# verificatum/verificatum-vmn

Hardware: AMD Instinct MI355X
Metric: modexps/sec (batched variable-base modPow, 2048-bit ModPGroup, full-length exponents) (higher is better)
Workload: dtype u32 limbs (28-bit radix), u64 accumulate

## Files before the change

__graft_entry__.py:

```python
from __future__ import annotations

import importlib.util
import os
import subprocess
import sys

ROOT = os.path.dirname(os.path.abspath(__file__))
PKG_DIR = os.path.join(ROOT, "verificatum-vmn_amd")
CSRC = os.path.join(PKG_DIR, "csrc")
LIB = os.path.join(PKG_DIR, "libvmnhip.so")
PROOFS_LIB = os.path.join(PKG_DIR, "libvmnproofs.so")


def load_package():
    name = "verificatum_vmn_amd"
    if name in sys.modules:
        return sys.modules[name]
    spec = importlib.util.spec_from_file_location(name, os.path.join(PKG_DIR, "__init__.py"),
                                                  submodule_search_locations=[PKG_DIR])
    mod = importlib.util.module_from_spec(spec)
    sys.modules[name] = mod
    spec.loader.exec_module(mod)
    return mod


def _newer(target: str, sources) -> bool:
    if not os.path.exists(target):
        return False
    t = os.path.getmtime(target)
    return all(os.path.getmtime(s) <= t for s in sources)


def build() -> None:
    hipcc = os.environ.get("HIPCC", "/opt/rocm/bin/hipcc")
    gspec = importlib.util.spec_from_file_location("gen_mont_asm", os.path.join(ROOT, "tools", "gen_mont_asm.py"))
    gmod = importlib.util.module_from_spec(gspec)
    gspec.loader.exec_module(gmod)
    gen = gmod.render([10, 14, 19, 37, 74], [110], [148, 76, 112], [80, 296], [592])
    inc = os.path.join(CSRC, "gen", "mont_rows.inc")
    inc29 = os.path.join(CSRC, "gen", "mont29_rows.inc")
    for path, text in ((inc, gen), (inc29, gmod.render29([71]))):
        if not os.path.exists(path) or open(path).read() != text:
            with open(path, "w") as f:
                f.write(text)
    units = ("vmnhip.hip", "inst_small.hip", "inst_2048.hip", "inst_2048_short.hip", "inst_2048_wide.hip", "inst_3072.hip", "inst_4096.hip", "inst_8192.hip",
             "inst_16384.hip", "inst_p224.hip", "inst_p256.hip", "inst_p384.hip", "inst_p521.hip",
             "inst_g9.hip", "inst_g10.hip", "inst_g13.hip", "inst_g15.hip", "inst_g21.hip")
    sources = [os.path.join(CSRC, f) for f in units + ("modp_kernels.h", "modp_shared_exp.h", "modp_instances.h", "ec_instances.h", "light_kernels.h", "ec_kernels.h", "mont28.h", "hostbig.h", "expprod_schedule.h", "ec_shared_schedule.h", "hexlines_layout.h", "jsonlines_layout.h", "decimal_kernels.h",
                                                       "vmnhip_internal.h", "sha256.h", "sha512.h", "hostnum64.h", "hosttrace.h")]
    sources += [inc, inc29, os.path.join(ROOT, "include", "vmnhip.h")]
    if not _newer(LIB, sources):
        objdir = os.path.join(CSRC, "build")
        os.makedirs(objdir, exist_ok=True)
        procs = []
        for u in units:
            obj = os.path.join(objdir, u.replace(".hip", ".o"))
            cmd = [hipcc, "-std=c++20", "-O3", "--offload-arch=gfx950", "-fPIC", "-c", os.path.join(CSRC, u), "-o", obj]
            procs.append((cmd, obj, subprocess.Popen(cmd)))
        objs = []
        for cmd, obj, pr in procs:
            if pr.wait() != 0:
                for _, _, other in procs:
                    if other.poll() is None:
                        other.kill()
                raise subprocess.CalledProcessError(pr.returncode, cmd)
            objs.append(obj)
        subprocess.run([hipcc, "--offload-arch=gfx950", "-shared", "-o", LIB] + objs, check=True)
    psrc = [os.path.join(CSRC, "vmnproofs.cpp"), os.path.join(CSRC, "hostnum64.h"), os.path.join(CSRC, "hostcurve.h"), os.path.join(CSRC, "hosttrace.h"),
            os.path.join(ROOT, "include", "vmnproofs.h"),
            os.path.join(ROOT, "include", "vmnhip.h"), LIB]
    if not _newer(PROOFS_LIB, psrc):
        subprocess.run(["g++", "-std=c++17", "-O2", "-Wall", "-pthread", "-fPIC", "-shared", os.path.join(CSRC, "vmnproofs.cpp"), "-o", PROOFS_LIB,
                        "-L" + PKG_DIR, "-lvmnhip", "-Wl,-rpath,$ORIGIN"], check=True)
    orc_dir = os.path.join(ROOT, "oracle")
    if not _newer(os.path.join(orc_dir, "libvmnoracle.so"), [os.path.join(orc_dir, "vmn_oracle.c")]):
        subprocess.run(["make", "-B", "-C", orc_dir, "libvmnoracle.so"], check=True,
                       stdout=subprocess.PIPE, stderr=subprocess.STDOUT)
    load_package()


def smoke() -> None:
    if ROOT not in sys.path:
        sys.path.insert(0, ROOT)
    vmn = load_package()
    from oracle import pyref
    from oracle.cbind import Oracle

    p, q, g = pyref.modp_group(2048)
    n = 512
    xs = [pow(1 + v % (p - 1), 2, p) for v in pyref.stream_ints(b"smoke/x", n, p)]
    es = pyref.stream_ints(b"smoke/e", n, q)
    ctx = vmn.Context(0)
    grp = vmn.ModPGroup(ctx, p, q, g)
    X = grp.toElementArray(xs)
    E = grp.ringArray(es)
    got = X.exp(E).toInts()
    orc = Oracle(p, q)
    want = orc.exp_array(xs, es)
    assert got == want, "smoke: HIP modpow differs from the GMP oracle"
    got_fixed = grp.exp(g, E).toInts()
    assert got_fixed == orc.exp_fixed(g, es), "smoke: HIP fixed-base exp differs from the GMP oracle"
# ... 40 lines not shown
```

verificatum-vmn_amd/csrc/modp_instances.h:

```cpp
#pragma once
#include "modp_kernels.h"
#include "modp_shared_exp.h"

#define VMN_MODP_INSTANCES(KW, S_, NW_, LPE_)                                                                                          \
    KW __global__ void vmn::k_import_be<vmn::Cfg<S_, LPE_>, NW_>(vmn::u32*, const uint8_t*, size_t, size_t, int, size_t, const vmn::u32*, \
                                                                 vmn::u32, const vmn::u32*, vmn::u32*);                                   \
    KW __global__ void vmn::k_export_be<vmn::Cfg<S_, LPE_>, NW_>(uint8_t*, size_t, size_t, int, const vmn::u32*, size_t, const vmn::u32*, \
                                                                 vmn::u32);                                                               \
    KW __global__ void vmn::k_to_words<vmn::Cfg<S_, LPE_>, NW_>(vmn::u32*, const vmn::u32*, size_t, const vmn::u32*, vmn::u32);           \
    KW __global__ void vmn::k_mul<vmn::Cfg<S_, LPE_>>(vmn::u32*, const vmn::u32*, const vmn::u32*, size_t, size_t, const vmn::u32*,      \
                                                      vmn::u32);                                                                         \
    KW __global__ void vmn::k_modpow<vmn::Cfg<S_, LPE_>>(vmn::u32*, const vmn::u32*, const vmn::u32*, int, size_t, int, int, size_t,     \
                                                         const vmn::u32*, vmn::u32, const vmn::u32*, vmn::u32*);                         \
    KW __global__ void vmn::k_modpow_phased<vmn::Cfg<S_, LPE_>>(vmn::u32*, const vmn::u32*, const vmn::u32*, int, size_t, int, int,      \
                                                                size_t, const vmn::u32*, vmn::u32, const vmn::u32*, vmn::u32*, int,      \
                                                                vmn::u32*, vmn::u32*);                                                   \
    KW __global__ void vmn::k_modpow2<vmn::Cfg<S_, LPE_>>(vmn::u32*, const vmn::u32*, const vmn::u32*, int, size_t, int, const vmn::u32*,  \
                                                          const vmn::u32*, int, size_t, int, int, size_t, const vmn::u32*, vmn::u32,      \
                                                          const vmn::u32*, vmn::u32*);                                                  \
    KW __global__ void vmn::k_modpow2_phased<vmn::Cfg<S_, LPE_>>(vmn::u32*, const vmn::u32*, const vmn::u32*, int, size_t, int,          \
                                                                 const vmn::u32*, const vmn::u32*, int, size_t, int, int, size_t,        \
                                                                 const vmn::u32*, vmn::u32, const vmn::u32*, vmn::u32*, int, vmn::u32*,  \
                                                                 vmn::u32*);                                                            \
    KW __global__ void vmn::k_modpow_shared<vmn::Cfg<S_, LPE_>>(vmn::u32*, const vmn::u32*, const vmn::SlideStep*, int, int, size_t,      \
                                                                const vmn::u32*, vmn::u32, vmn::u32*);                                  \
    KW __global__ void vmn::k_modpow_shared_phased<vmn::Cfg<S_, LPE_>>(vmn::u32*, const vmn::u32*, const vmn::SlideStep*, int, int,      \
                                                                       size_t, const vmn::u32*, vmn::u32, vmn::u32*, int, vmn::u32*,     \
                                                                       vmn::u32*);                                                      \
    KW __global__ void vmn::k_modpow_shared_multi<vmn::Cfg<S_, LPE_>>(vmn::SharedArrays, vmn::u32, vmn::u32, const vmn::SlideStep*, int,  \
                                                                      int, size_t, const vmn::u32*, vmn::u32, vmn::u32*);              \
    KW __global__ void vmn::k_modpow_shared_multi_phased<vmn::Cfg<S_, LPE_>>(vmn::SharedArrays, vmn::u32, vmn::u32,                     \
                                                                             const vmn::SlideStep*, int, int, size_t, const vmn::u32*,  \
                                                                             vmn::u32, vmn::u32*, int, vmn::u32*, vmn::u32*);           \
    KW __global__ void vmn::k_modpow_shared_each<vmn::Cfg<S_, LPE_>>(vmn::EachArrays, vmn::u32, vmn::u32, const vmn::SlideStep*, int,     \
                                                                     size_t, const vmn::u32*, vmn::u32, vmn::u32*);                    \
    KW __global__ void vmn::k_modpow_shared_each_phased<vmn::Cfg<S_, LPE_>>(vmn::EachArrays, vmn::u32, vmn::u32, const vmn::SlideStep*,  \
                                                                            int, size_t, const vmn::u32*, vmn::u32, vmn::u32*, int,    \
                                                                            vmn::u32*, vmn::u32*);                                     \
    KW __global__ void vmn::k_modpow_expprod<vmn::Cfg<S_, LPE_>>(vmn::ExpProdArrays, vmn::u32, vmn::u32, const vmn::SlideStep*, vmn::u32,    \
                                                                 const vmn::u32*, vmn::u32, vmn::u32*);                                \
    KW __global__ void vmn::k_modpow_jobs<vmn::Cfg<S_, LPE_>>(vmn::ModpowJob, vmn::ModpowJob, unsigned, int, const vmn::u32*, vmn::u32,    \
                                                              const vmn::u32*, vmn::u32*);                                             \
    KW __global__ void vmn::k_reduce_strided<vmn::Cfg<S_, LPE_>, true>(vmn::u32*, const vmn::u32*, size_t, size_t, size_t,               \
                                                                       const vmn::u32*, vmn::u32);                                       \
    KW __global__ void vmn::k_reduce_strided<vmn::Cfg<S_, LPE_>, false>(vmn::u32*, const vmn::u32*, size_t, size_t, size_t,              \
                                                                        const vmn::u32*, vmn::u32);                                      \
    KW __global__ void vmn::k_ring_elementwise<vmn::Cfg<S_, LPE_>>(vmn::u32*, const vmn::u32*, const vmn::u32*, const vmn::u32*, int,    \
                                                                   size_t, const vmn::u32*, vmn::u32);                                   \
    KW __global__ void vmn::k_scan_totals<vmn::Cfg<S_, LPE_>, true>(vmn::u32*, const vmn::u32*, const vmn::u32*, size_t, size_t, size_t, \
                                                                    int, const vmn::u32*, vmn::u32, const vmn::u32*);                    \
    KW __global__ void vmn::k_scan_totals<vmn::Cfg<S_, LPE_>, false>(vmn::u32*, const vmn::u32*, const vmn::u32*, size_t, size_t, size_t, \
                                                                     int, const vmn::u32*, vmn::u32, const vmn::u32*);                   \
    KW __global__ void vmn::k_scan_apply<vmn::Cfg<S_, LPE_>>(vmn::u32*, const vmn::u32*, const vmn::u32*, const vmn::u32*, size_t,       \
                                                             size_t, size_t, int, const vmn::u32*, vmn::u32, const vmn::u32*);           \
    KW __global__ void vmn::k_fixed_level<vmn::Cfg<S_, LPE_>>(vmn::u32*, int, int, int, const vmn::u32*, vmn::u32);                      \
    KW __global__ void vmn::k_fixed_exp<vmn::Cfg<S_, LPE_>>(vmn::u32*, const vmn::u32*, int, int, const vmn::u32*, int, size_t, int,     \
                                                            const vmn::u32*, vmn::u32);                                                  \
    KW __global__ void vmn::k_bucket_level<vmn::Cfg<S_, LPE_>, true>(vmn::u32*, size_t, vmn::LevelInputs, unsigned, const vmn::u32*,     \
                                                                     const vmn::u32*, const vmn::u32*, const vmn::u32*, size_t, size_t, \
                                                                     vmn::u32, const vmn::u32*, vmn::u32);                               \
    KW __global__ void vmn::k_bucket_level<vmn::Cfg<S_, LPE_>, false>(vmn::u32*, size_t, vmn::LevelInputs, unsigned, const vmn::u32*,    \
                                                                      const vmn::u32*, const vmn::u32*, const vmn::u32*, size_t, size_t, \
                                                                      vmn::u32, const vmn::u32*, vmn::u32);

#define VMN_MEMBER_INSTANCE_ONE_LANE(KW, S_, LPE_) \
    KW __global__ void vmn::k_jacobi_member<vmn::Cfg<S_, LPE_>>(const vmn::u32*, size_t, const vmn::u32*, vmn::u32*);
#define VMN_MEMBER_INSTANCE_LANES(KW, S_, LPE_) \
    KW __global__ void vmn::k_jacobi_member_lanes<vmn::Cfg<S_, LPE_>>(const vmn::u32*, size_t, const vmn::u32*, vmn::u32*);

#define VMN_UNIT_SMALL(KW)                                                                                             \
    VMN_MODP_INSTANCES(KW, 10, 8, 1) VMN_MODP_INSTANCES(KW, 14, 12, 1) VMN_MODP_INSTANCES(KW, 19, 16, 1)                 \
    VMN_MODP_INSTANCES(KW, 37, 32, 1) VMN_MEMBER_INSTANCE_ONE_LANE(KW, 10, 1) VMN_MEMBER_INSTANCE_ONE_LANE(KW, 14, 1)     \
    VMN_MEMBER_INSTANCE_ONE_LANE(KW, 19, 1) VMN_MEMBER_INSTANCE_ONE_LANE(KW, 37, 1)
#define VMN_UNIT_2048(KW) VMN_MODP_INSTANCES(KW, 74, 64, 1) VMN_MEMBER_INSTANCE_ONE_LANE(KW, 74, 1)
#define VMN_UNIT_2048_SHORT(KW)                                                                                        \
    KW __global__ void vmn::k_modpow<vmn::Cfg<74, 1>, true>(vmn::u32*, const vmn::u32*, const vmn::u32*, int, size_t, int, int, size_t, \
                                                            const vmn::u32*, vmn::u32, const vmn::u32*, vmn::u32*);                     \
    KW __global__ void vmn::k_modpow_phased<vmn::Cfg<74, 1>, true>(vmn::u32*, const vmn::u32*, const vmn::u32*, int, size_t, int, int,  \
                                                                   size_t, const vmn::u32*, vmn::u32, const vmn::u32*, vmn::u32*, int,  \
                                                                   vmn::u32*, vmn::u32*);
#define VMN_UNIT_2048_WIDE(KW)                                                                                         \
    VMN_MODP_INSTANCES(KW, 76, 64, 4) VMN_MODP_INSTANCES(KW, 80, 64, 8)                                                \
    KW __global__ void vmn::k_modpow_jobs_mixed<vmn::Cfg<80, 8>, vmn::Cfg<76, 4>>(vmn::ModpowJob, vmn::ModpowJob, unsigned, int,       \
                                                                                 const vmn::u32*, vmn::u32, const vmn::u32*, vmn::u32*);
#define VMN_UNIT_3072(KW) VMN_MODP_INSTANCES(KW, 110, 96, 2) VMN_MODP_INSTANCES(KW, 112, 96, 4) VMN_MEMBER_INSTANCE_LANES(KW, 110, 2)
#define VMN_UNIT_4096(KW) VMN_MODP_INSTANCES(KW, 148, 128, 4) VMN_MEMBER_INSTANCE_LANES(KW, 148, 4)
#define VMN_UNIT_8192(KW) VMN_MODP_INSTANCES(KW, 296, 256, 8) VMN_MEMBER_INSTANCE_LANES(KW, 296, 8)
#define VMN_UNIT_16384(KW) VMN_MODP_INSTANCES(KW, 592, 512, 16) VMN_MEMBER_INSTANCE_LANES(KW, 592, 16)
```

verificatum-vmn_amd/csrc/vmnhip.hip:

```cpp
#include <stdarg.h>

#include <algorithm>
#include <future>
#include <memory>
#include <system_error>
#include <utility>

#include "ec_kernels.h"
#include "modp_kernels.h"
#include "modp_instances.h"
#include "ec_instances.h"
#include "light_kernels.h"
#include "decimal_kernels.h"
#include "vmnhip_internal.h"
#include "sha256.h"
#include "sha512.h"
#include "hostnum64.h"
#include "ec_shared_schedule.h"
#include "expprod_schedule.h"
#include "hexlines_layout.h"

VMN_UNIT_SMALL(extern template)
VMN_UNIT_2048(extern template)
VMN_UNIT_2048_SHORT(extern template)
VMN_UNIT_2048_WIDE(extern template)
VMN_UNIT_3072(extern template)
VMN_UNIT_4096(extern template)
VMN_UNIT_8192(extern template)
VMN_UNIT_16384(extern template)
VMN_UNIT_P224(extern template)
VMN_UNIT_P256(extern template)
VMN_UNIT_P384(extern template)
VMN_UNIT_P521(extern template)
VMN_UNIT_G9(extern template)
VMN_UNIT_G10(extern template)
VMN_UNIT_G13(extern template)
VMN_UNIT_G15(extern template)
VMN_UNIT_G21(extern template)

using namespace vmn;
using vmn::hostbig::Big;

static thread_local char g_err[512] = "";
void vmn::set_error(const char* fmt, ...) {
    va_list ap;
    va_start(ap, fmt);
    vsnprintf(g_err, sizeof(g_err), fmt, ap);
    va_end(ap);
}
extern "C" const char* vmn_last_error(void) { return g_err; }
static thread_local vmn_ctx* tl_helper_of = nullptr;
vmn_ctx* vmn::lane_of(vmn_ctx* c) { return (c && tl_helper_of == c && c->helper) ? c->helper : c; }
extern "C" void vmn_report_error(const char* message) { vmn::set_error("%s", message ? message : ""); }
extern "C" const char* vmn_version(void) { return "vmnhip 0.1 (gfx950, radix-2^28 lazy-carry Montgomery)"; }

#define ARG_CHECK(cond, msg)             \
    do {                                 \
        if (!(cond)) {                   \
// ... 26 lines not shown
static int with_curve(const vmn_modulus& m, F&& f) {
#define X(S_, NW_, K_) \
    if (m.ec->S == S_ && m.ec->kind == K_) return f(CurveCfg<S_, NW_, K_>{});
    VMN_FOR_CURVES(X)
#undef X
    return VMN_ERR_ARG;
}

static bool size_for_bits(int nbits, int* S, int* NW, int* LPE) {
    const int sizes[][4] = {{256, 10, 8, 1}, {384, 14, 12, 1}, {512, 19, 16, 1}, {1024, 37, 32, 1}, {2048, 74, 64, 1},
                            {3072, 110, 96, 2}, {4096, 148, 128, 4}, {8192, 296, 256, 8}, {16384, 592, 512, 16}};
    for (auto& s : sizes) {
        if (nbits <= s[0]) {
            *S = s[1];
            *NW = s[2];
            *LPE = s[3];
            return true;
        }
    }
    return false;
}

static size_t default_wide_max() {
    static const size_t v = [] {
        const char* env = getenv("VMN_WIDE_MAX");
        return env ? (size_t)strtoull(env, nullptr, 10) : (size_t)40960;
    }();
    return v;
}
static size_t default_wide8_max() {
    static const size_t v = [] {
        const char* env = getenv("VMN_WIDE8_MAX");
        return env ? (size_t)strtoull(env, nullptr, 10) : (size_t)6144;
    }();
    return v;
}
static size_t fixed_split_fill() {
    const char* env = getenv("VMN_FIXED_SPLIT_FILL");
    return env ? (size_t)strtoull(env, nullptr, 10) : (size_t)786432;
}
static const vmn_modulus& geom(const vmn_ctx* ctx, const vmn_modulus& m, size_t items, bool always = false) {
    const vmn_ctx* root = ctx->parent ? ctx->parent : ctx;
    if (m.wide8 && root->wide8_max != 0 && (items <= root->wide8_max || (always && items <= root->wide_max))) return *m.wide8;
    if (!m.wide || root->wide_max == 0) return m;
    return (always || items <= root->wide_max) ? *m.wide : m;
}
template <class F>
static int with_geom(const vmn_ctx* ctx, const vmn_modulus& m0, size_t items, F&& f, bool always = false) {
    const vmn_modulus& m = geom(ctx, m0, items, always);
    return with_cfg(m, [&](auto c, auto w) { return f(c, w, m); });
}
static size_t lds_bytes(const vmn_modulus& m) { return (size_t)m.S * (BLOCK / m.LPE) * sizeof(u32); }
static int blocks_per_cu(const vmn_modulus&) { return 2; }

template <typename... KArgs, typename... Args>
static int launch_timed(vmn_ctx* ctx, const char* family, void (*kernel)(KArgs...), unsigned grid, size_t lds, Args... args) {
    TimingRec rec;
    if (ctx->timing) {
        rec.family = family;
        rec.mads = ctx->next_mads;
        rec.canon = ctx->next_canon;
        VMN_HIP(hipEventCreate(&rec.start));
        VMN_HIP(hipEventCreate(&rec.stop));
        VMN_HIP(hipEventRecord(rec.start, ctx->stream));
    }
    ctx->next_mads = ctx->next_canon = 0;
    hipLaunchKernelGGL(kernel, dim3(grid), dim3(BLOCK), lds, ctx->stream, static_cast<KArgs>(args)...);
    VMN_HIP(hipGetLastError());
    if (ctx->timing) {
        VMN_HIP(hipEventRecord(rec.stop, ctx->stream));
        ctx->recs.push_back(rec);
    }
    return VMN_OK;
}
template <typename... KArgs, typename... Args>
static int launch(vmn_ctx* ctx, const char* family, void (*kernel)(KArgs...), unsigned grid, size_t lds, Args... args) {
    const void* kp = reinterpret_cast<const void*>(kernel);
    if (!ctx->lds_attr_set.count(kp)) {
        VMN_HIP(hipFuncSetAttribute(kp, hipFuncAttributeMaxDynamicSharedMemorySize, (int)lds));
        ctx->lds_attr_set.insert(kp);
    }
    return launch_timed(ctx, family, kernel, grid, lds, args...);
}

static void note_work(vmn_ctx* ctx, const vmn_modulus& m, double products, double squarings = 0, double canon_products = -1) {
    if (!ctx->timing) return;
    const double S = m.ec ? (double)m.ec->S : (double)m.S;
    const double Rw = m.ec ? S : (double)m.rows;
    const double s32 = (double)((m.nbits + 31) / 32);
    ctx->next_canon = (canon_products >= 0 ? canon_products : products) * (2 * s32 * s32 + s32) +
                      squarings * (m.ec ? 2 * s32 * s32 + s32 : s32 * (s32 + 1) / 2 + s32 * s32 + s32);
    if (m.ec) {
        const bool known = m.ec->kind == EC_NIST;
        const double nz = known && m.ec->S == 10 ? 7 : known && m.ec->S == 15 ? 12 : S;
        ctx->next_mads = (products + squarings) * (S * S + S * nz);
        return;
    }
    const double sq = Rw * S + Rw * (S + SQR_BLK * m.LPE) / 2;
    ctx->next_mads = products * 2 * Rw * S + squarings * sq;
}
static const double EC_ADD = 15.4, EC_MADD = 10.6, EC_DBL = 6.9, EC_NORM = 7.0, EC_INV = 380;
static const double EC_MADD_RUN = 9.7;

static unsigned light_grid(vmn_ctx* ctx, size_t work_items) {
    size_t blocks = (work_items + BLOCK - 1) / BLOCK;
    size_t cap = (size_t)ctx->num_cus * 8;
// ... 1338 lines not shown
    int phases = 1;
    DevTmp tab, sync_words;
    PhasePlan(vmn_ctx* ctx, const vmn_modulus& m, size_t n, size_t arrays = 1)
        : max_blocks((unsigned)(ctx->num_cus * blocks_per_cu(m))), epb((size_t)(BLOCK / m.LPE)), ntiles(arrays * ((n + epb - 1) / epb)),
          tab(ctx), sync_words(ctx) {
        if (const char* mb = getenv("VMN_MODPOW_MAX_BLOCKS")) {
            const int v = atoi(mb);
            if (v >= 1) max_blocks = std::min<unsigned>(max_blocks, (unsigned)v);
        }
        grid = (unsigned)std::min<size_t>(ntiles, max_blocks);
    }
    size_t slot_tables_bytes(const vmn_modulus& m, size_t rows) const { return (size_t)grid * epb * rows * elem_words(m) * sizeof(uint32_t); }
    int split(vmn_ctx* ctx, const vmn_modulus& m, int cuttable_steps, size_t rows) {
        static const int phases_env = [] {
            const char* e = getenv("VMN_MODPOW_PHASES");
            return e && *e ? std::max(1, atoi(e)) : 16;
        }();
        if (ntiles <= (size_t)max_blocks || ntiles >= ((size_t)1 << 26)) return VMN_OK;
        const int want = std::min(phases_env, std::max(1, cuttable_steps));
        const size_t tab_bytes = ntiles * epb * rows * elem_words(m) * sizeof(uint32_t);
        if (want == 1 || tab_bytes > ((size_t)64 << 30) || tab.alloc(tab_bytes) != VMN_OK) return VMN_OK;
        VMN_TRY(sync_words.alloc((ntiles + 1) * sizeof(uint32_t)));
        VMN_TRY(dev_zero(ctx, sync_words.p, (ntiles + 1) * sizeof(uint32_t)));
        phases = want;
        return VMN_OK;
    }
    uint32_t* table() { return tab.as<uint32_t>(); }
    uint32_t* queue() { return sync_words.as<uint32_t>(); }
    uint32_t* done() { return queue() + 1; }
};

static int modpow_words(vmn_ctx* ctx, const vmn_modulus& m0, const uint32_t* x, const uint32_t* e_words, int ewords,
                        size_t estride, int ebits, size_t n, uint32_t* out) {
    if (n == 0) return VMN_OK;
    if (ebits < 1) ebits = 1;
    if (m0.ec) {
        const vmn_modulus& m = m0;
        int wb = std::min(pick_window(ebits), 5);
        unsigned grid = std::min<unsigned>(grid_for(n), (unsigned)(ctx->num_cus * 2));
        size_t tab_bytes = (size_t)grid * BLOCK * ((size_t)1 << wb) * elem_words(m) * sizeof(uint32_t);
        VMN_TRY(ensure_scratch(ctx, tab_bytes));
        note_work(ctx, m, (double)n * (EC_DBL * ebits + EC_ADD * ((ebits + wb - 1) / wb + (1 << wb))));
        return with_curve(m, [&]<class E>(E) {
            return launch_light(ctx, "modpow", k_ec_mulvar<E::S, E::KIND>, grid, out, x, e_words, ewords, estride, ebits, wb, n, ecdev(m.ec),
                                reinterpret_cast<uint32_t*>(ctx->scratch));
        });
    }
    int wbits = pick_window(ebits);
    const vmn_modulus& m = geom(ctx, m0, n);
    const int nwin = (ebits + wbits - 1) / wbits;
    PhasePlan pl(ctx, m, n);
    VMN_TRY(ensure_scratch(ctx, pl.slot_tables_bytes(m, (size_t)1 << wbits)));
    note_work(ctx, m, (double)n * (nwin - 1 + (1 << wbits) - 2), (double)n * (nwin - 1) * wbits);
    const bool pow29 = m.S == 74 && m.LPE == 1;
    const char* short_env = getenv("VMN_POW29_SHORT");
    const bool pow29_short = pow29 && m.pow29_short && !(short_env && *short_env && atoi(short_env) == 0);
    if (pow29 && ctx->timing) {
        const double S9 = Cfg29::S, relief = 2 * (S9 - 2), red = S9 * (pow29_short ? S9 - 2 : S9);
        ctx->next_mads = (double)n * ((nwin - 1 + (1 << wbits) - 2 + 2) * (S9 * S9 + red + relief) +
                                      (double)(nwin - 1) * wbits * (red + S9 * (S9 + SQR_BLK) / 2 + relief));
    }
    VMN_TRY(pl.split(ctx, m, nwin - 1, (size_t)1 << wbits));
    static_assert(POW29<Cfg<74, 1>>, "modpow_words passes the 29-bit constants to the kernels of Cfg<74, 1>");
    const uint32_t* d_n = pow29 ? m.d_pow29 + (size_t)(pow29_short ? Cfg29::ROW_NS : Cfg29::ROW_N) * Cfg29::W : m.d_n;
    const uint32_t* d_one = pow29 ? m.d_pow29 + (size_t)Cfg29::ROW_ONE * Cfg29::W : m.d_one;
    const uint32_t n0inv = pow29 ? m.n0inv29 : m.n0inv;
    if (pow29_short) {
        using C = Cfg<74, 1>;
        if (pl.phases > 1)
            return launch(ctx, "modpow", k_modpow_phased<C, true>, pl.max_blocks, lds_bytes(m), out, x, e_words, ewords, estride, ebits,
                          wbits, n, d_n, n0inv, d_one, pl.table(), pl.phases, pl.queue(), pl.done());
        return launch(ctx, "modpow", k_modpow<C, true>, pl.grid, lds_bytes(m), out, x, e_words, ewords, estride, ebits, wbits, n, d_n,
                      n0inv, d_one, reinterpret_cast<uint32_t*>(ctx->scratch));
    }
    return with_cfg(m, [&]<class C, class W>(C, W) {
        if (pl.phases > 1)
            return launch(ctx, "modpow", k_modpow_phased<C>, pl.max_blocks, lds_bytes(m), out, x, e_words, ewords, estride, ebits, wbits, n,
                          d_n, n0inv, d_one, pl.table(), pl.phases, pl.queue(), pl.done());
        return launch(ctx, "modpow", k_modpow<C>, pl.grid, lds_bytes(m), out, x, e_words, ewords, estride, ebits, wbits, n, d_n, n0inv,
                      d_one, reinterpret_cast<uint32_t*>(ctx->scratch));
    });
}

static int sliding_window_bits(int ebits) {
    if (const char* env = getenv("VMN_SLIDING_WINDOW")) {
        int w = atoi(env);
        if (w >= 0 && w <= 8) return w;
    }
    int best = 2;
    long best_cost = 1L << 60;
    for (int w = 2; w <= 8; ++w) {
        long cost = (1L << (w - 1)) + ebits / (w + 1);
        if (cost < best_cost) {
            best_cost = cost;
            best = w;
        }
    }
    return best;
}
static void slide_schedule(const Big& e, int ebits, int w, std::vector<SlideStep>& steps, long& mults, long& squarings) {
    const size_t first = steps.size();
    int pending = 0;
    mults = squarings = 0;
    for (int i = ebits - 1; i >= 0;) {
        if (!hostbig::get_bit(e, i)) {
            ++pending;
            --i;
            continue;
        }
        int l = std::max(i - w + 1, 0);
        while (!hostbig::get_bit(e, l)) ++l;
        uint32_t val = 0;
        for (int b = i; b >= l; --b) val = (val << 1) | (uint32_t)hostbig::get_bit(e, b);
        steps.push_back(SlideStep{steps.size() == first ? 0 : pending + (i - l + 1), (int)((val - 1) / 2)});
        pending = 0;
        i = l - 1;
    }
    if (pending) steps.push_back(SlideStep{pending, -1});
// ... 2482 lines not shown
                                   (int)chain, ecdev(m.ec));
                return hipGetLastError() == hipSuccess ? VMN_OK : VMN_ERR_DEVICE;
            });
        }
        if (rc == VMN_OK)
            rc = launch_light(ctx, "fixed_table", k_fixed_seed, grid_for((size_t)nwin * (w + 1)), ft.d_tab,
                              (const uint32_t*)sq.as<uint32_t>(), w, nwin, (const uint32_t*)m.d_one, (int)Wd);
        for (int l = 1; l < w && rc == VMN_OK; ++l) {
            size_t lanes = (((size_t)1 << l) - 1) * nwin;
            rc = with_curve(m, [&]<class E>(E) {
                note_work(ctx, m, EC_ADD * (double)lanes);
                return launch_light(ctx, "fixed_table", k_ec_fixed_level<E::S, E::KIND>, grid_for(lanes), ft.d_tab, w, nwin, l, ecdev(m.ec));
            });
        }
        free_one(ctx, m, d_base);
        if (rc == VMN_OK) {
            DevTmp flat(ctx);
            const size_t entries = (size_t)nwin << w;
            rc = flat.alloc(entries * Wd * sizeof(uint32_t));
            const uint32_t* whole[1] = {ft.d_tab};
            if (rc == VMN_OK) rc = ec_normalize(ctx, m, whole, 1, entries, flat.as<uint32_t>());
            if (rc == VMN_OK && hipMemcpyAsync(ft.d_tab, flat.p, entries * Wd * sizeof(uint32_t), hipMemcpyDeviceToDevice, ctx->stream) != hipSuccess)
                rc = VMN_ERR_DEVICE;
        }
        if (rc != VMN_OK) {
            if (ft.d_tab) (void)hipFree(ft.d_tab);
            return rc;
        }
        ft.last_use = ++g->fixed_clock;
        ft.uses = carry_uses;
        ft.built_on = ctx->stream;
        if (hipEventCreateWithFlags(&ft.ready, hipEventDisableTiming) == hipSuccess) (void)hipEventRecord(ft.ready, ctx->stream);
        g->fixed_bytes += ft.bytes;
        auto ins = g->fixed.emplace(key, ft);
        *out = &ins.first->second;
        return VMN_OK;
    }
    VMN_TRACE("fixed_table:build");
    const size_t chain = (size_t)nwin * w;
    std::vector<uint8_t> own_chain;
    if (!chain_be || chain_be->size() != (chain + 1) * g->nbytes) {
        VMN_TRY(fixed_chain_host(g, base_be, chain, own_chain));
        chain_be = &own_chain;
    }
    const std::vector<uint8_t>& sq_be = *chain_be;
    DevTmp sq(ctx);
    VMN_TRY(sq.alloc((chain + 1) * Wd * sizeof(uint32_t)));
    int ok = 1;
    VMN_TRY(import_be(ctx, m, g->nbytes, sq_be.data(), chain + 1, sq.as<uint32_t>(), &ok));
    VMN_TRY(mul_arrays(ctx, m, sq.as<uint32_t>(), sq.as<uint32_t>() + chain * Wd, 0, chain, sq.as<uint32_t>()));
    vmn_group::FixedTable ft;
    ft.wbits = w;
    ft.nwin = nwin;
    ft.bytes = (size_t)nwin * ((size_t)1 << w) * Wd * sizeof(uint32_t);
    VMN_TRY(fixed_alloc(g, ft.bytes, &ft.d_tab));
    int rc = launch_light(ctx, "fixed_table", k_fixed_seed, grid_for((size_t)nwin * (w + 1)), ft.d_tab, (const uint32_t*)sq.as<uint32_t>(), w,
                          nwin, (const uint32_t*)m.d_one, (int)Wd);
    for (int l = 1; l < w && rc == VMN_OK; ++l) {
        size_t lanes = (((size_t)1 << l) - 1) * nwin;
        rc = with_geom(ctx, m, lanes, [&]<class C, class W>(C, W, const vmn_modulus& mg) {
            note_work(ctx, mg, (double)lanes);
            return launch(ctx, "fixed_table", k_fixed_level<C>, egrid(mg, lanes), lds_bytes(mg), ft.d_tab, w, nwin, l, mg.d_n, mg.n0inv);
        });
    }
    if (rc != VMN_OK) {
        (void)hipFree(ft.d_tab);
        return rc;
    }
    ft.last_use = ++g->fixed_clock;
    ft.uses = carry_uses;
    ft.built_on = ctx->stream;
    if (hipEventCreateWithFlags(&ft.ready, hipEventDisableTiming) == hipSuccess) (void)hipEventRecord(ft.ready, ctx->stream);
    g->fixed_bytes += ft.bytes;
    auto ins = g->fixed.emplace(key, ft);
    *out = &ins.first->second;
    return VMN_OK;
}

extern "C" int vmn_group_precompute_fixed(vmn_group* grp, const uint8_t* base_be, size_t n_hint, int uses_hint) {
    ARG_CHECK(grp && base_be && n_hint > 0, "bad argument");
    const int uses = uses_hint < 1 ? 1 : (uses_hint > 16 ? 16 : uses_hint);
    const int ebits = grp->Q.nbits;
    vmn_group::FixedTable* ft = nullptr;
    std::vector<uint8_t> chain;
    if (!grp->P.ec) {
        {
            VMN_ENTER(LANE(grp->ctx));
            std::lock_guard<std::recursive_mutex> tab_guard(grp->tab_mu);
            VMN_TRY(fixed_table(grp, base_be, ebits, n_hint, &ft, uses, true));
            if (ft) return VMN_OK;
        }
        const int w = fixed_window_for(grp, n_hint, ebits, uses);
        VMN_TRY(fixed_chain_host(grp, base_be, (size_t)((ebits + w - 1) / w) * w, chain));
    }
    VMN_ENTER(LANE(grp->ctx));
    std::lock_guard<std::recursive_mutex> tab_guard(grp->tab_mu);
    return fixed_table(grp, base_be, ebits, n_hint, &ft, uses, false, chain.empty() ? nullptr : &chain);
}

extern "C" int vmn_group_release_fixed(vmn_group* grp, const uint8_t* base_be) {
    ARG_CHECK(grp && base_be, "null argument");
    VMN_ENTER(LANE(grp->ctx));
    std::lock_guard<std::recursive_mutex> tab_guard(grp->tab_mu);
    std::string key(reinterpret_cast<const char*>(base_be), grp->P.ec ? 2 * grp->nbytes : grp->nbytes);
    auto it = grp->fixed.find(key);
    if (it != grp->fixed.end()) fixed_drop(grp, it);
    return VMN_OK;
}

extern "C" int vmn_group_exp_fixed(vmn_group* grp, const uint8_t* base_be, const vmn_rarray* e, vmn_garray** out) {
    ARG_CHECK(grp && base_be && e && out, "null argument");
    ARG_CHECK(e->grp == grp, "exponent array belongs to another group");
    vmn_ctx* ctx = LANE(grp->ctx);
    VMN_ENTER(ctx);
    const size_t n = e->n;
    vmn_garray* r = nullptr;
    VMN_TRY(new_garray(grp, n, &r));
    if (n == 0) {
        *out = r;
        return VMN_OK;
    }
    int ebits = grp->Q.nbits;
    vmn_group::FixedTable* ft = nullptr;
    DevTmp ew(ctx);
    std::lock_guard<std::recursive_mutex> tab_guard(grp->tab_mu);
    int rc = fixed_table(grp, base_be, ebits, n, &ft);
    if (rc == VMN_OK) rc = ew.alloc(n * (size_t)grp->Q.NW * sizeof(uint32_t));
    if (rc == VMN_OK) rc = to_words(ctx, grp->Q, e->d, n, ew.as<uint32_t>());
    if (rc == VMN_OK && grp->P.ec) {
        const vmn_modulus& m = grp->P;
        rc = with_curve(m, [&]<class E>(E) {
            note_work(ctx, m, EC_MADD_RUN * (double)n * (ft->nwin - 1), 0, EC_MADD * (double)n * (ft->nwin - 1));
            return launch_light(ctx, "fixed", k_ec_fixed_exp<E::S, E::KIND>, grid_for(n), r->d, (const uint32_t*)ft->d_tab, ft->wbits, ft->nwin,
                                (const uint32_t*)ew.as<uint32_t>(), grp->Q.NW, n, ecdev(m.ec));
        });
    } else if (rc == VMN_OK) {
        int parts = 1;
        const size_t fill = fixed_split_fill();
        while (parts < 16 && (size_t)(2 * parts) * n <= fill && ft->nwin / (2 * parts) >= 4) parts *= 2;
        const size_t items = n * (size_t)parts, Wd = elem_words(grp->P);
        const vmn_modulus& m = geom(ctx, grp->P, items);
        DevTmp pieces(ctx);
        if (parts > 1) rc = pieces.alloc(items * Wd * sizeof(uint32_t));
        uint32_t* dst = parts > 1 ? pieces.as<uint32_t>() : r->d;
        unsigned grid = egrid(m, items);
        if (rc == VMN_OK) {
            rc = with_cfg(m, [&]<class C, class W>(C, W) {
                note_work(ctx, m, (double)n * (ft->nwin - parts));
                return launch(ctx, "fixed", k_fixed_exp<C>, grid, lds_bytes(m), dst, (const uint32_t*)ft->d_tab, ft->wbits, ft->nwin,
                              (const uint32_t*)ew.as<uint32_t>(), grp->Q.NW, n, parts, m.d_n, m.n0inv);
            });
        }
        for (int half = parts / 2; half >= 1 && rc == VMN_OK; half /= 2) {
            uint32_t* lo = pieces.as<uint32_t>();
            rc = mul_arrays(ctx, grp->P, lo, lo + (size_t)half * n * Wd, Wd, (size_t)half * n, half == 1 ? r->d : lo);
        }
    }
    if (rc != VMN_OK) {
        vmn_garray_free(r);
        return rc;
    }
    *out = r;
    return VMN_OK;
}

static int ec_normalize(vmn_ctx* ctx, const vmn_modulus& m, const uint32_t* const* ins, size_t k, size_t n, uint32_t* out) {
    if (n == 0 || k == 0) return VMN_OK;
    const char* K_str = getenv("VMN_EC_NORMALISE_CHUNK");
    const size_t K_env = K_str && *K_str ? (size_t)std::max(2, atoi(K_str)) : (size_t)0;
    const size_t FWd = (size_t)stride_for_limbs(m.ec->S), Wd = (size_t)m.W, K = K_env ? K_env : 8, TOP = 2048;
    const size_t n1 = (n + K - 1) / K;
    std::vector<size_t> sizes{k * n, k * n1};
    while (sizes.back() > TOP) sizes.push_back((sizes.back() + K - 1) / K);
    const size_t L = sizes.size();
    size_t words = 0;
    std::vector<size_t> off_pref(L), off_val(L), off_inv(L);
    for (size_t l = 0; l < L; ++l) {
        off_pref[l] = words;
        words += (l + 1 < L ? sizes[l] : 0) * FWd;
        off_val[l] = words;
        words += (l > 0 ? sizes[l] : 0) * FWd;
        off_inv[l] = words;
        words += (l > 0 ? sizes[l] : 0) * FWd;
    }
    DevTmp buf(ctx);
    VMN_TRY(buf.alloc(words * sizeof(uint32_t)));
    uint32_t* B = buf.as<uint32_t>();
    double products = 7.0 * (double)(k * n) + EC_INV * (double)sizes[L - 1];
    for (size_t l = 1; l + 1 < L; ++l) products += 3.0 * (double)sizes[l];
    return with_curve(m, [&]<class E>(E) -> int {
        constexpr int S = E::S, KIND = E::KIND;
        note_work(ctx, m, products);
        const unsigned bpa = (unsigned)((n1 + BLOCK - 1) / BLOCK);
        for (size_t a0 = 0; a0 < k; a0 += LEVEL_ARRAYS) {
            const size_t ga = std::min<size_t>(LEVEL_ARRAYS, k - a0);
            LevelInputs li{};
            for (size_t a = 0; a < ga; ++a) li.p[a] = ins[a0 + a];
            VMN_TRY(launch_light(ctx, "normalize", k_finv_up<S, true, KIND>, (unsigned)(bpa * ga), B + off_pref[0] + a0 * n * FWd,
                                 B + off_val[1] + a0 * n1 * FWd, li, bpa, n, K, ecdev(m.ec)));
// ... 577 lines not shown
```

verificatum-vmn_amd/csrc/vmnhip_internal.h:

```cpp
#pragma once
#include <hip/hip_runtime.h>
#include <stdint.h>
#include <stdio.h>
#include <string.h>
#include <map>
#include <mutex>
#include <string>
#include <unordered_set>
#include <vector>

#include "../../include/vmnhip.h"
#include "hostbig.h"
#include "hostnum64.h"
#include "hostcurve.h"
#include "hosttrace.h"

struct vmn_ctx;
namespace vmn {

void set_error(const char* fmt, ...);

#define VMN_HIP(call)                                                                         \
    do {                                                                                      \
        hipError_t err__ = (call);                                                            \
// ... 82 lines not shown
    const uint32_t* d_one = nullptr;
    const uint32_t* d_rr = nullptr;
    const uint32_t* d_b = nullptr;
    const uint32_t* d_a = nullptr;
    int a_zero = 0;
    const uint32_t* d_mp = nullptr;
    const uint32_t* d_mp2 = nullptr;
    const uint32_t* d_pm2 = nullptr;
    const uint32_t* d_pp14 = nullptr;
    uint32_t n0inv = 0;
    vmn::num64::Mod* f64 = nullptr;
    vmn::num64::HostCurve host;
    vmn::num64::Num rd_inv;
    uint32_t p1p = 0;
    int ts_s = 0, ts_ewords = 0;
    const uint32_t* d_ts_e = nullptr;
    const uint32_t* d_ts_c = nullptr;
};

struct vmn_modulus {
    int S = 0;
    int NW = 0;
    int LPE = 1;
    int rows = 0;
    vmn_modulus* wide = nullptr;
    vmn_modulus* wide8 = nullptr;
    int W = 0;
    const vmn_curve* ec = nullptr;
    int nbits = 0;
    uint32_t n0inv = 0;
    uint32_t* d_n = nullptr;
    uint32_t* d_rr = nullptr;
    uint32_t* d_one = nullptr;
    uint32_t* d_pow29 = nullptr;
    uint32_t n0inv29 = 0;
    bool pow29_short = false;
    vmn::hostbig::Big n_words;
    vmn::hostbig::Mont* hm = nullptr;
    vmn::num64::Mod* hm64 = nullptr;
};

struct vmn_group {
    vmn_ctx* ctx = nullptr;
    vmn_curve* curve = nullptr;
    size_t nbytes = 0;
    size_t xbytes = 0;
    vmn_modulus P;
    vmn_modulus Q;
    vmn::hostbig::Big g_words;
    struct FixedTable {
        uint32_t* d_tab = nullptr;
        int wbits = 0;
        int nwin = 0;
        size_t bytes = 0;
        uint64_t last_use = 0;
        int uses = 0;
        hipEvent_t ready = nullptr;
        hipStream_t built_on = nullptr;
    };
    std::map<std::string, FixedTable> fixed;
    std::recursive_mutex tab_mu;
    size_t fixed_bytes = 0;
    uint64_t fixed_clock = 0;
    struct DecimalTables {
        uint32_t* d_pow10 = nullptr;
        uint32_t* d_pow2 = nullptr;
        uint32_t dmax = 0;
        uint32_t nc = 0;
        uint32_t nwa = 0;
        uint32_t nw = 0;
    };
    DecimalTables dec;
};

struct vmn_garray {
    vmn_group* grp = nullptr;
    uint32_t* d = nullptr;
    size_t n = 0;
    size_t bytes = 0;
    vmn_ctx* lane = nullptr;
};

struct vmn_rarray {
    vmn_group* grp = nullptr;
    uint32_t* d = nullptr;
    size_t n = 0;
    size_t bytes = 0;
    vmn_ctx* lane = nullptr;
};
```

Before: 1.744 million.

## Build and use fixed-base exponentiation tables in 29-bit Montgomery form

Adds 29-bit radix kernels for fixed-base table construction (enter, level doubling) and fixed-base exponentiation for 2048-bit groups, reusing the pow29 constants already used by variable-base modpow. The table is kept in 29-bit Montgomery form and the result is converted back on store. This targets the cost of fixed-base exp, not the measured variable-base modPow path, so the benchmark metric is unlikely to change. It adds an env toggle and more kernel instances, which raise compile time and code size.

New measurement: 1.743 million, median of 2. Within noise of the previous version (-0.1%).

```diff
diff --git a/__graft_entry__.py b/__graft_entry__.py
--- a/__graft_entry__.py
+++ b/__graft_entry__.py
@@ -46,7 +46,7 @@
     units = ("vmnhip.hip", "inst_small.hip", "inst_2048.hip", "inst_2048_short.hip", "inst_2048_wide.hip", "inst_3072.hip", "inst_4096.hip", "inst_8192.hip",
              "inst_16384.hip", "inst_p224.hip", "inst_p256.hip", "inst_p384.hip", "inst_p521.hip",
              "inst_g9.hip", "inst_g10.hip", "inst_g13.hip", "inst_g15.hip", "inst_g21.hip")
-    sources = [os.path.join(CSRC, f) for f in units + ("modp_kernels.h", "modp_shared_exp.h", "modp_instances.h", "ec_instances.h", "light_kernels.h", "ec_kernels.h", "mont28.h", "hostbig.h", "expprod_schedule.h", "ec_shared_schedule.h", "hexlines_layout.h", "jsonlines_layout.h", "decimal_kernels.h",
+    sources = [os.path.join(CSRC, f) for f in units + ("modp_kernels.h", "modp_shared_exp.h", "modp_fixed29.h", "modp_instances.h", "ec_instances.h", "light_kernels.h", "ec_kernels.h", "mont28.h", "hostbig.h", "expprod_schedule.h", "ec_shared_schedule.h", "hexlines_layout.h", "jsonlines_layout.h", "decimal_kernels.h",
                                                        "vmnhip_internal.h", "sha256.h", "sha512.h", "hostnum64.h", "hosttrace.h")]
     sources += [inc, inc29, os.path.join(ROOT, "include", "vmnhip.h")]
     if not _newer(LIB, sources):
diff --git a/verificatum-vmn_amd/csrc/modp_fixed29.h b/verificatum-vmn_amd/csrc/modp_fixed29.h
--- /dev/null
+++ b/verificatum-vmn_amd/csrc/modp_fixed29.h
@@ -0,0 +1,93 @@
+#pragma once
+#include "modp_kernels.h"
+
+namespace vmn {
+
+template <bool SHORT>
+__global__ void __launch_bounds__(BLOCK, Cfg29T<SHORT>::MINW)
+k_fixed29_enter(u32* __restrict__ rows, size_t n, const u32* __restrict__ nmod, u32 n0inv, const u32* __restrict__ one_m) {
+    using C = Cfg<74, 1>;
+    using K = Cfg29T<SHORT>;
+    constexpr int W = K::W;
+    extern __shared__ u32 lds[];
+    Lane<K> ln(lds);
+    u32 nn[K::L];
+    load_modulus<K>(nn, nmod, ln);
+    size_t el = (size_t)blockIdx.x * K::EPB + ln.eslot;
+    bool live = el < n;
+    size_t ec = live ? el : n - 1;
+    u32 a[K::L];
+    {
+        u32 x[C::L];
+        load_elem<C>(x, rows + ec * W, Lane<C>(lds));
+        repack_limbs<K::L, K::BITS, C::L, C::BITS>(a, x);
+    }
+    const_to_lds<K>(ln, one_m + (Cfg29::ROW_CIN - Cfg29::ROW_ONE) * W);
+    mont_mul<K>(a, a, ln, nn, n0inv);
+    if (live) store_elem<K>(rows + el * W, a, ln);
+}
+
+template <bool SHORT>
+__global__ void __launch_bounds__(BLOCK, Cfg29T<SHORT>::MINW)
+k_fixed29_level(u32* __restrict__ T, int w, int nwin, int l, const u32* __restrict__ nmod, u32 n0inv) {
+    using K = Cfg29T<SHORT>;
+    constexpr int W = K::W;
+    extern __shared__ u32 lds[];
+    Lane<K> ln(lds);
+    u32 nn[K::L];
+    load_modulus<K>(nn, nmod, ln);
+    size_t per = ((size_t)1 << l) - 1;
+    size_t t = (size_t)blockIdx.x * K::EPB + ln.eslot;
+    bool live = t < per * nwin;
+    size_t tc = live ? t : per * nwin - 1;
+    size_t k = tc / per, r = tc % per + 1;
+    u32* row = T + (k << w) * W;
+    u32 a[K::L];
+    load_elem<K>(a, row + r * W, ln);
+    load_elem_to_lds<K>(ln, row + ((size_t)1 << l) * W);
+    u32 o[K::L];
+    mont_mul<K>(o, a, ln, nn, n0inv);
+    if (live) store_elem<K>(row + (((size_t)1 << l) + r) * W, o, ln);
+}
+
+template <bool SHORT>
+__global__ void __launch_bounds__(BLOCK, Cfg29T<SHORT>::MINW)
+k_fixed29_exp(u32* __restrict__ out, const u32* __restrict__ T, int w, int nwin, const u32* __restrict__ e, int ewords,
+              size_t n, int parts, const u32* __restrict__ nmod, u32 n0inv, const u32* __restrict__ one_m) {
+    using C = Cfg<74, 1>;
+    using K = Cfg29T<SHORT>;
+    constexpr int W = K::W;
+    extern __shared__ u32 lds[];
+    Lane<K> ln(lds);
+    u32 nn[K::L];
+    load_modulus<K>(nn, nmod, ln);
+    const size_t items = n * (size_t)parts;
+    const size_t ntiles = (items + K::EPB - 1) / K::EPB;
+    for (size_t t = blockIdx.x; t < ntiles; t += gridDim.x) {
+        size_t it = t * K::EPB + ln.eslot;
+        bool live = it < items;
+        size_t ic = live ? it : items - 1;
+        const int part = (int)(ic / n);
+        const size_t ec = ic % n;
+        const int k0 = (int)((long)part * nwin / parts), k1 = (int)((long)(part + 1) * nwin / parts);
+        const u32* ep = e + ec * ewords;
+        u32 a[K::L];
+        u32 d = exp_digit(ep, ewords, k0 * w, w);
+        load_elem<K>(a, T + (((size_t)k0 << w) + d) * W, ln);
+#pragma unroll 1
+        for (int k = k0 + 1; k < k1; ++k) {
+            d = exp_digit(ep, ewords, k * w, w);
+            load_elem_to_lds<K>(ln, T + (((size_t)k << w) + d) * W);
+            mont_mul<K>(a, a, ln, nn, n0inv);
+        }
+        pow29_store<C, K>(out + it * W, a, true, live, one_m, ln, nn, n0inv);
+    }
+}
+
+}
+
+#define VMN_FIXED29_INSTANCES(KW, SHORT_)                                                                                   \
+    KW __global__ void vmn::k_fixed29_enter<SHORT_>(vmn::u32*, size_t, const vmn::u32*, vmn::u32, const vmn::u32*);          \
+    KW __global__ void vmn::k_fixed29_level<SHORT_>(vmn::u32*, int, int, int, const vmn::u32*, vmn::u32);                    \
+    KW __global__ void vmn::k_fixed29_exp<SHORT_>(vmn::u32*, const vmn::u32*, int, int, const vmn::u32*, int, size_t, int,   \
+                                                  const vmn::u32*, vmn::u32, const vmn::u32*);
diff --git a/verificatum-vmn_amd/csrc/modp_instances.h b/verificatum-vmn_amd/csrc/modp_instances.h
--- a/verificatum-vmn_amd/csrc/modp_instances.h
+++ b/verificatum-vmn_amd/csrc/modp_instances.h
@@ -1,6 +1,7 @@
 #pragma once
 #include "modp_kernels.h"
 #include "modp_shared_exp.h"
+#include "modp_fixed29.h"
 
 #define VMN_MODP_INSTANCES(KW, S_, NW_, LPE_)                                                                                          \
     KW __global__ void vmn::k_import_be<vmn::Cfg<S_, LPE_>, NW_>(vmn::u32*, const uint8_t*, size_t, size_t, int, size_t, const vmn::u32*, \
@@ -72,13 +73,14 @@
     VMN_MODP_INSTANCES(KW, 10, 8, 1) VMN_MODP_INSTANCES(KW, 14, 12, 1) VMN_MODP_INSTANCES(KW, 19, 16, 1)                 \
     VMN_MODP_INSTANCES(KW, 37, 32, 1) VMN_MEMBER_INSTANCE_ONE_LANE(KW, 10, 1) VMN_MEMBER_INSTANCE_ONE_LANE(KW, 14, 1)     \
     VMN_MEMBER_INSTANCE_ONE_LANE(KW, 19, 1) VMN_MEMBER_INSTANCE_ONE_LANE(KW, 37, 1)
-#define VMN_UNIT_2048(KW) VMN_MODP_INSTANCES(KW, 74, 64, 1) VMN_MEMBER_INSTANCE_ONE_LANE(KW, 74, 1)
+#define VMN_UNIT_2048(KW) VMN_MODP_INSTANCES(KW, 74, 64, 1) VMN_MEMBER_INSTANCE_ONE_LANE(KW, 74, 1) VMN_FIXED29_INSTANCES(KW, false)
 #define VMN_UNIT_2048_SHORT(KW)                                                                                        \
     KW __global__ void vmn::k_modpow<vmn::Cfg<74, 1>, true>(vmn::u32*, const vmn::u32*, const vmn::u32*, int, size_t, int, int, size_t, \
                                                             const vmn::u32*, vmn::u32, const vmn::u32*, vmn::u32*);                     \
     KW __global__ void vmn::k_modpow_phased<vmn::Cfg<74, 1>, true>(vmn::u32*, const vmn::u32*, const vmn::u32*, int, size_t, int, int,  \
                                                                    size_t, const vmn::u32*, vmn::u32, const vmn::u32*, vmn::u32*, int,  \
-                                                                   vmn::u32*, vmn::u32*);
+                                                                   vmn::u32*, vmn::u32*);                                               \
+    VMN_FIXED29_INSTANCES(KW, true)
 #define VMN_UNIT_2048_WIDE(KW)                                                                                         \
     VMN_MODP_INSTANCES(KW, 76, 64, 4) VMN_MODP_INSTANCES(KW, 80, 64, 8)                                                \
     KW __global__ void vmn::k_modpow_jobs_mixed<vmn::Cfg<80, 8>, vmn::Cfg<76, 4>>(vmn::ModpowJob, vmn::ModpowJob, unsigned, int,       \
diff --git a/verificatum-vmn_amd/csrc/vmnhip.hip b/verificatum-vmn_amd/csrc/vmnhip.hip
--- a/verificatum-vmn_amd/csrc/vmnhip.hip
+++ b/verificatum-vmn_amd/csrc/vmnhip.hip
@@ -4,6 +4,7 @@
 #include <future>
 #include <memory>
 #include <system_error>
+#include <type_traits>
 #include <utility>
 
 #include "ec_kernels.h"
@@ -136,6 +137,28 @@
 }
 static size_t lds_bytes(const vmn_modulus& m) { return (size_t)m.S * (BLOCK / m.LPE) * sizeof(u32); }
 static int blocks_per_cu(const vmn_modulus&) { return 2; }
+
+struct Pow29Rows {
+    bool on = false;
+    bool short_rows = false;
+    const uint32_t* d_n(const vmn_modulus& m) const { return m.d_pow29 + (size_t)(short_rows ? Cfg29::ROW_NS : Cfg29::ROW_N) * Cfg29::W; }
+    const uint32_t* d_one(const vmn_modulus& m) const { return m.d_pow29 + (size_t)Cfg29::ROW_ONE * Cfg29::W; }
+    double product_mads() const {
+        const double S9 = Cfg29::S;
+        return S9 * S9 + S9 * (short_rows ? S9 - 2 : S9) + 2 * (S9 - 2);
+    }
+};
+template <class F>
+static int with_rows29(const Pow29Rows& r, F&& f) {
+    return r.short_rows ? f(std::true_type{}) : f(std::false_type{});
+}
+static Pow29Rows pow29_rows(const vmn_modulus& m) {
+    Pow29Rows r;
+    r.on = m.S == 74 && m.LPE == 1 && !m.ec;
+    const char* short_env = getenv("VMN_POW29_SHORT");
+    r.short_rows = r.on && m.pow29_short && !(short_env && *short_env && atoi(short_env) == 0);
+    return r;
+}
 
 template <typename... KArgs, typename... Args>
 static int launch_timed(vmn_ctx* ctx, const char* family, void (*kernel)(KArgs...), unsigned grid, size_t lds, Args... args) {
@@ -1580,18 +1603,17 @@
     PhasePlan pl(ctx, m, n);
     VMN_TRY(ensure_scratch(ctx, pl.slot_tables_bytes(m, (size_t)1 << wbits)));
     note_work(ctx, m, (double)n * (nwin - 1 + (1 << wbits) - 2), (double)n * (nwin - 1) * wbits);
-    const bool pow29 = m.S == 74 && m.LPE == 1;
-    const char* short_env = getenv("VMN_POW29_SHORT");
-    const bool pow29_short = pow29 && m.pow29_short && !(short_env && *short_env && atoi(short_env) == 0);
+    const Pow29Rows p29 = pow29_rows(m);
+    const bool pow29 = p29.on, pow29_short = p29.short_rows;
     if (pow29 && ctx->timing) {
         const double S9 = Cfg29::S, relief = 2 * (S9 - 2), red = S9 * (pow29_short ? S9 - 2 : S9);
-        ctx->next_mads = (double)n * ((nwin - 1 + (1 << wbits) - 2 + 2) * (S9 * S9 + red + relief) +
+        ctx->next_mads = (double)n * ((nwin - 1 + (1 << wbits) - 2 + 2) * p29.product_mads() +
                                       (double)(nwin - 1) * wbits * (red + S9 * (S9 + SQR_BLK) / 2 + relief));
     }
     VMN_TRY(pl.split(ctx, m, nwin - 1, (size_t)1 << wbits));
     static_assert(POW29<Cfg<74, 1>>, "modpow_words passes the 29-bit constants to the kernels of Cfg<74, 1>");
-    const uint32_t* d_n = pow29 ? m.d_pow29 + (size_t)(pow29_short ? Cfg29::ROW_NS : Cfg29::ROW_N) * Cfg29::W : m.d_n;
-    const uint32_t* d_one = pow29 ? m.d_pow29 + (size_t)Cfg29::ROW_ONE * Cfg29::W : m.d_one;
+    const uint32_t* d_n = pow29 ? p29.d_n(m) : m.d_n;
+    const uint32_t* d_one = pow29 ? p29.d_one(m) : m.d_one;
     const uint32_t n0inv = pow29 ? m.n0inv29 : m.n0inv;
     if (pow29_short) {
         using C = Cfg<74, 1>;
@@ -4180,12 +4202,34 @@
     vmn_group::FixedTable ft;
     ft.wbits = w;
     ft.nwin = nwin;
+    const char* f29_env = getenv("VMN_FIXED29");
+    const Pow29Rows p29 = pow29_rows(geom(ctx, m, n));
+    ft.form29 = p29.on && !(f29_env && *f29_env && atoi(f29_env) == 0);
     ft.bytes = (size_t)nwin * ((size_t)1 << w) * Wd * sizeof(uint32_t);
     VMN_TRY(fixed_alloc(g, ft.bytes, &ft.d_tab));
-    int rc = launch_light(ctx, "fixed_table", k_fixed_seed, grid_for((size_t)nwin * (w + 1)), ft.d_tab, (const uint32_t*)sq.as<uint32_t>(), w,
-                          nwin, (const uint32_t*)m.d_one, (int)Wd);
+    int rc = VMN_OK;
+    if (ft.form29) {
+        note_work(ctx, m, (double)chain);
+        if (ctx->timing) ctx->next_mads = (double)chain * p29.product_mads();
+        rc = with_rows29(p29, [&](auto s) {
+            return launch(ctx, "fixed_table", k_fixed29_enter<decltype(s)::value>, egrid(m, chain), lds_bytes(m), sq.as<uint32_t>(), chain,
+                          p29.d_n(m), m.n0inv29, p29.d_one(m));
+        });
+    }
+    if (rc == VMN_OK)
+        rc = launch_light(ctx, "fixed_table", k_fixed_seed, grid_for((size_t)nwin * (w + 1)), ft.d_tab, (const uint32_t*)sq.as<uint32_t>(), w,
+                          nwin, ft.form29 ? p29.d_one(m) : (const uint32_t*)m.d_one, (int)Wd);
     for (int l = 1; l < w && rc == VMN_OK; ++l) {
         size_t lanes = (((size_t)1 << l) - 1) * nwin;
+        if (ft.form29) {
+            note_work(ctx, m, (double)lanes);
+            if (ctx->timing) ctx->next_mads = (double)lanes * p29.product_mads();
+            rc = with_rows29(p29, [&](auto s) {
+                return launch(ctx, "fixed_table", k_fixed29_level<decltype(s)::value>, egrid(m, lanes), lds_bytes(m), ft.d_tab, w, nwin, l,
+                              p29.d_n(m), m.n0inv29);
+            });
+            continue;
+        }
         rc = with_geom(ctx, m, lanes, [&]<class C, class W>(C, W, const vmn_modulus& mg) {
             note_work(ctx, mg, (double)lanes);
             return launch(ctx, "fixed_table", k_fixed_level<C>, egrid(mg, lanes), lds_bytes(mg), ft.d_tab, w, nwin, l, mg.d_n, mg.n0inv);
@@ -4267,12 +4311,20 @@
         const size_t fill = fixed_split_fill();
         while (parts < 16 && (size_t)(2 * parts) * n <= fill && ft->nwin / (2 * parts) >= 4) parts *= 2;
         const size_t items = n * (size_t)parts, Wd = elem_words(grp->P);
-        const vmn_modulus& m = geom(ctx, grp->P, items);
+        const vmn_modulus& m = ft->form29 ? grp->P : geom(ctx, grp->P, items);
         DevTmp pieces(ctx);
         if (parts > 1) rc = pieces.alloc(items * Wd * sizeof(uint32_t));
         uint32_t* dst = parts > 1 ? pieces.as<uint32_t>() : r->d;
         unsigned grid = egrid(m, items);
-        if (rc == VMN_OK) {
+        if (rc == VMN_OK && ft->form29) {
+            const Pow29Rows p29 = pow29_rows(m);
+            note_work(ctx, m, (double)n * ft->nwin, 0, (double)n * (ft->nwin - parts));
+            if (ctx->timing) ctx->next_mads = (double)n * ft->nwin * p29.product_mads();
+            rc = with_rows29(p29, [&](auto s) {
+                return launch(ctx, "fixed", k_fixed29_exp<decltype(s)::value>, grid, lds_bytes(m), dst, (const uint32_t*)ft->d_tab, ft->wbits,
+                              ft->nwin, (const uint32_t*)ew.as<uint32_t>(), grp->Q.NW, n, parts, p29.d_n(m), m.n0inv29, p29.d_one(m));
+            });
+        } else if (rc == VMN_OK) {
             rc = with_cfg(m, [&]<class C, class W>(C, W) {
                 note_work(ctx, m, (double)n * (ft->nwin - parts));
                 return launch(ctx, "fixed", k_fixed_exp<C>, grid, lds_bytes(m), dst, (const uint32_t*)ft->d_tab, ft->wbits, ft->nwin,
diff --git a/verificatum-vmn_amd/csrc/vmnhip_internal.h b/verificatum-vmn_amd/csrc/vmnhip_internal.h
--- a/verificatum-vmn_amd/csrc/vmnhip_internal.h
+++ b/verificatum-vmn_amd/csrc/vmnhip_internal.h
@@ -158,6 +158,7 @@
         uint32_t* d_tab = nullptr;
         int wbits = 0;
         int nwin = 0;
+        bool form29 = false;
         size_t bytes = 0;
         uint64_t last_use = 0;
         int uses = 0;
```
